# zju-pi/diff-sampler

Hardware: AMD Instinct MI355X
Metric: images/sec (whole node) at NFE=10, EDM CIFAR-10 (higher is better)
Workload: dtype fp32; 1 GPU; EDM CIFAR-10 32x32 SongUNet (55.7M params), DPM-Solver++(2M) logSNR NFE=10, batch 256/GPU; launch=eager

## Files before the change

### diff_sampler_amd/csrc/conv3x3_wino.hip

```cpp
#include <type_traits>

#include "igemm_common.h"

namespace igemm {
namespace {

typedef float f32x2 __attribute__((ext_vector_type(2)));

constexpr int WV_NO_NORM = 2, WV_NO_HALO = 4, WV_NO_DMA = 8, WV_NO_EPI = 16;
constexpr int WINO_K = 8;
constexpr int WINO_POS = 2 * 64 * 4;
constexpr int WINO_IMG = 16 * WINO_POS;
constexpr int WINO_NSH = 4;
constexpr int WINO_EPI_LD = 36;

#define DS_WINO_WAIT_VM0() do { __builtin_amdgcn_s_waitcnt(0x0F70); asm volatile("" ::: "memory"); } while (0)

template <int VAR, int NORM, int NSL>
__global__ void __launch_bounds__(256, 1) conv3x3_wino_kernel(const KParams p) {
    extern __shared__ __attribute__((aligned(16))) float smem[];
    float* Us = smem;
    float* Vs = smem + 2 * WINO_IMG;
    float* Hs = Vs + WINO_IMG;

    const int tid = threadIdx.x, lane = tid & 63;
    const int wave = __builtin_amdgcn_readfirstlane(tid >> 6);
    const int wr = wave >> 1, wc = wave & 1;
    int mt, nt;
    if (!decode_tile(blockIdx.x, p.mtiles, p.ntiles, mt, nt)) return;
    const int m0 = mt * 256, n0 = nt * 64;
    const int img0 = m0 / p.HW;
    const int r0 = (m0 - img0 * p.HW) / p.W;
    const int WPH = p.WP >> 1, Wt = p.W >> 1;
    const int Ctot = p.c0 + p.c1;
    const int nslabs = Ctot / WINO_K;
    constexpr bool kDma = !(VAR & WV_NO_DMA), kHalo = !(VAR & WV_NO_HALO);
    constexpr int kNorm = (VAR & WV_NO_NORM) ? 0 : NORM;

    const int kh_h = tid & 1;
    unsigned h_off0[WINO_NSH], h_off1[WINO_NSH];
    int h_lds[WINO_NSH];
    bool h_ok[WINO_NSH];
#pragma unroll
    for (int j = 0; j < WINO_NSH; ++j) {
        const int hp = (tid + j * 256) >> 1;
        const int hr = hp / p.WP, hc = hp - hr * p.WP;
        const int y = r0 + hr - 1, x = hc - 1;
        const bool in = hp < p.NP;
        h_ok[j] = in && (unsigned)y < (unsigned)p.H && (unsigned)x < (unsigned)p.W;
        const int pix = min(max(y, 0), p.H - 1) * p.W + min(max(x, 0), p.W - 1);
        h_off0[j] = (unsigned)(pix * p.lda0 + kh_h * 4);
        h_off1[j] = (unsigned)(pix * p.lda1 + kh_h * 4);
        h_lds[j] = in ? (((kh_h * 2 + (hc & 1)) * p.HP + hr) * WPH + (hc >> 1)) * 4 : p.NP * WINO_K;
    }
    const float* a0i = p.a0 + (size_t)img0 * p.HW * p.lda0;
    const float* a1i = p.a1 + (size_t)img0 * p.HW * p.lda1;
    const float* cpi = p.norm + (size_t)img0 * 3 * Ctot + kh_h * 4;
    f32x4 hreg[WINO_NSH];
    float h_t[4 * WINO_NSH], h_u[4 * WINO_NSH];
    f32x4 cmu = {0.f, 0.f, 0.f, 0.f}, cga = {1.f, 1.f, 1.f, 1.f}, cbe = {0.f, 0.f, 0.f, 0.f};
    const float* h_src = nullptr;
    unsigned h_sel = 0;
    auto halo_src = [&](int s) {
        const int c = s * WINO_K;
        const bool first = c < p.c0;
        h_src = first ? a0i + c : a1i + (c - p.c0);
        h_sel = (unsigned)__builtin_amdgcn_readfirstlane(first ? -1 : 0);
        asm volatile("" : "+s"(h_sel));
    };
    auto halo_load1 = [&](auto J) {
        constexpr int j = decltype(J)::value;
        if constexpr (j >= NSL) return;
        const unsigned off = (h_off0[j] & h_sel) | (h_off1[j] & ~h_sel);
        hreg[j] = *reinterpret_cast<const f32x4*>(h_src + off);
    };
    auto coef_load1 = [&](int s, auto I) {
        constexpr int i = decltype(I)::value;
        if constexpr (NORM != 0) {
            const f32x4 v = *reinterpret_cast<const f32x4*>(cpi + (size_t)i * Ctot + s * WINO_K);
            if constexpr (i == 0) cmu = v; else if constexpr (i == 1) cga = v; else cbe = v;
        }
    };
    auto halo_chain = [&](auto C, auto ST) {
        constexpr int c = decltype(C)::value, st = decltype(ST)::value, j = c >> 2, e = c & 3;
        if constexpr (j >= NSL) return;
        if constexpr (st == 0 && kNorm != 0) {
            h_t[c] = __builtin_fmaf(hreg[j][e] - cmu[e], cga[e], cbe[e]);
            if constexpr (kNorm == 2) h_u[c] = __expf(-h_t[c]);
        }
        if constexpr (st == 1 && kNorm == 2) h_u[c] = __builtin_amdgcn_rcpf(1.0f + h_u[c]);
        if constexpr (st == 2) {
            float v = hreg[j][e];
            if constexpr (kNorm == 1) v = h_t[c];
            if constexpr (kNorm == 2) v = h_t[c] * h_u[c];
            hreg[j][e] = h_ok[j] ? v : 0.f;
            if constexpr (e == 3) *reinterpret_cast<f32x4*>(Hs + h_lds[j]) = hreg[j];
        }
    };

    const int t_t = (tid >> 1) & 63, cpl = tid & 1, kh_t = tid >> 7;
    const int t_ty = t_t / Wt, t_tx = t_t - t_ty * Wt;
    const float* h_rd = Hs + ((kh_t * 2 * p.HP + 2 * t_ty) * WPH + t_tx) * 4 + cpl * 2;
    const int h_par = p.HP * WPH * 4;
    float* v_wr = Vs + (kh_t * 64 + t_t) * 4 + cpl * 2;
    auto transform = [&]() {
        f32x2 d[4][4];
#pragma unroll
        for (int i = 0; i < 4; ++i)
#pragma unroll
            for (int j = 0; j < 4; ++j)
                d[i][j] = *reinterpret_cast<const f32x2*>(h_rd + (j & 1) * h_par + i * WPH * 4 + (j >> 1) * 4);
        DS_RACE_SKEW(wave);
        f32x2 t[4][4];
#pragma unroll
        for (int j = 0; j < 4; ++j) {
            t[0][j] = d[0][j] - d[2][j];
            t[1][j] = d[1][j] + d[2][j];
            t[2][j] = d[2][j] - d[1][j];
            t[3][j] = d[1][j] - d[3][j];
        }
#pragma unroll
        for (int i = 0; i < 4; ++i) {
            *reinterpret_cast<f32x2*>(v_wr + (i * 4 + 0) * WINO_POS) = t[i][0] - t[i][2];
            *reinterpret_cast<f32x2*>(v_wr + (i * 4 + 1) * WINO_POS) = t[i][1] + t[i][2];
            *reinterpret_cast<f32x2*>(v_wr + (i * 4 + 2) * WINO_POS) = t[i][2] - t[i][1];
            *reinterpret_cast<f32x2*>(v_wr + (i * 4 + 3) * WINO_POS) = t[i][1] - t[i][3];
        }
    };

    const float* u_src = p.b + (size_t)nt * nslabs * WINO_IMG + tid * 4;
    auto u_dma1 = [&](const float* src, float* ubuf, auto I) {
        constexpr int i = decltype(I)::value;
        float* dst = ubuf + (i * 256 + wave * 64) * 4;
        typedef const __attribute__((address_space(1))) void* gptr_t;
        typedef __attribute__((address_space(3))) void* lptr_t;
        __builtin_amdgcn_global_load_lds((gptr_t)(src + i * 1024), (lptr_t)(dst), 16, 0, 0);
    };

    f32x16 acc[16];
#pragma unroll
    for (int q = 0; q < 16; ++q)
#pragma unroll
        for (int r = 0; r < 16; ++r) acc[q][r] = 0.f;
    const int a_off = ((lane >> 5) * 64 + wr * 32 + (lane & 31)) * 4;
    const int b_off = ((lane >> 5) * 64 + wc * 32 + (lane & 31)) * 4;

#define DS_WINO_I(n) std::integral_constant<int, (n)>{}
#define DS_WINO_EACH4(F) F(0) F(1) F(2) F(3)
#define DS_WINO_EACH16(F, b) F((b) + 0) F((b) + 1) F((b) + 2) F((b) + 3) F((b) + 4) F((b) + 5) F((b) + 6) F((b) + 7)                \
                             F((b) + 8) F((b) + 9) F((b) + 10) F((b) + 11) F((b) + 12) F((b) + 13) F((b) + 14) F((b) + 15)

    halo_src(0);
#define DS_WINO_F(j) halo_load1(DS_WINO_I(j));
    DS_WINO_EACH4(DS_WINO_F)
#undef DS_WINO_F
    coef_load1(0, DS_WINO_I(0)); coef_load1(0, DS_WINO_I(1)); coef_load1(0, DS_WINO_I(2));
    DS_RACE_SKEW(wave);
#define DS_WINO_F(i) u_dma1(u_src, Us, DS_WINO_I(i)); u_dma1(u_src, Us, DS_WINO_I((i) + 4));
    DS_WINO_EACH4(DS_WINO_F)
#undef DS_WINO_F
    DS_RACE_SKEW(wave);
#define DS_WINO_F(c) halo_chain(DS_WINO_I(c), DS_WINO_I(0)); halo_chain(DS_WINO_I(c), DS_WINO_I(1)); halo_chain(DS_WINO_I(c), DS_WINO_I(2));
    DS_WINO_EACH16(DS_WINO_F, 0)
#undef DS_WINO_F
    {
        const int s1 = min(1, nslabs - 1);
        halo_src(s1);
#define DS_WINO_F(j) halo_load1(DS_WINO_I(j));
        DS_WINO_EACH4(DS_WINO_F)
#undef DS_WINO_F
        coef_load1(s1, DS_WINO_I(0)); coef_load1(s1, DS_WINO_I(1)); coef_load1(s1, DS_WINO_I(2));
    }
    DS_WINO_WAIT_VM0();
    __syncthreads();

    f32x4 fa[2][4], fb[2][4];
    int s = 0;
    do {
        const float* ub = Us + (s & 1) * WINO_IMG;
        transform();
        __syncthreads();
        const int s1 = min(s + 1, nslabs - 1), s2 = min(s + 2, nslabs - 1);
        const float* un = u_src + (size_t)s1 * WINO_IMG;
        float* ubn = Us + ((s + 1) & 1) * WINO_IMG;
        if constexpr (kHalo) halo_src(s2);
        auto frag_read = [&](auto G, auto I) {
            constexpr int g = decltype(G)::value, i = decltype(I)::value;
            if constexpr (i < 4) fa[g & 1][i] = *reinterpret_cast<const f32x4*>(Vs + (g * 4 + i) * WINO_POS + a_off);
            else fb[g & 1][i - 4] = *reinterpret_cast<const f32x4*>(ub + (g * 4 + i - 4) * WINO_POS + b_off);
        };
        if constexpr (kHalo) {
            DS_RACE_SKEW(wave);
#define DS_WINO_F(c) halo_chain(DS_WINO_I(c), DS_WINO_I(0)); halo_chain(DS_WINO_I(c), DS_WINO_I(1)); halo_chain(DS_WINO_I(c), DS_WINO_I(2));
            DS_WINO_EACH16(DS_WINO_F, 0)
#undef DS_WINO_F
        }
        auto fill = [&](auto K) {
            constexpr int k = decltype(K)::value, g = k >> 4;
            if constexpr (k < 8) {
                if constexpr (kDma) {
                    if constexpr (k == 0) DS_RACE_SKEW(wave);
                    u_dma1(un, ubn, DS_WINO_I(k));
                }
            } else if constexpr (k < 12) {
                if constexpr (kHalo) halo_load1(DS_WINO_I(k - 8));
            } else if constexpr (k < 15) {
                if constexpr (kHalo) coef_load1(s2, DS_WINO_I(k - 12));
            }
            constexpr int fr = g == 0 ? 8 : g == 1 ? 20 : g == 2 ? 32 : 64;
            if constexpr (k >= fr && k < fr + 8) frag_read(DS_WINO_I(g + 1), DS_WINO_I(k - fr));
        };
#define DS_WINO_STEP(k)                                                                                                                \
        acc[((k) >> 4) * 4 + ((k) & 3)] = __builtin_amdgcn_mfma_f32_32x32x2f32(fa[((k) >> 4) & 1][(k) & 3][((k) >> 2) & 3],            \
                                                                               fb[((k) >> 4) & 1][(k) & 3][((k) >> 2) & 3],            \
                                                                               acc[((k) >> 4) * 4 + ((k) & 3)], 0, 0, 0);              \
        fill(DS_WINO_I(k));                                                                                                            \
        __builtin_amdgcn_sched_barrier(0);
#define DS_WINO_F(i) frag_read(DS_WINO_I(0), DS_WINO_I(i)); frag_read(DS_WINO_I(0), DS_WINO_I((i) + 4));
        DS_WINO_EACH4(DS_WINO_F)
#undef DS_WINO_F
        __builtin_amdgcn_sched_barrier(0);
        DS_WINO_EACH16(DS_WINO_STEP, 0)
        DS_WINO_EACH16(DS_WINO_STEP, 16)
        DS_WINO_EACH16(DS_WINO_STEP, 32)
        DS_WINO_EACH16(DS_WINO_STEP, 48)
#undef DS_WINO_STEP
        DS_WINO_WAIT_VM0();
        __syncthreads();
    } while (++s < nslabs);
#undef DS_WINO_EACH16
#undef DS_WINO_EACH4
#undef DS_WINO_I

    if constexpr ((VAR & WV_NO_EPI) != 0) {
#pragma unroll
        for (int q = 0; q < 16; ++q) asm volatile("" :: "v"(acc[q]));
        return;
    }

    f32x16 Y[4];
#pragma unroll
    for (int a = 0; a < 2; ++a) {
        f32x16 t[4];
#pragma unroll
        for (int j = 0; j < 4; ++j) t[j] = a == 0 ? acc[j] + acc[4 + j] + acc[8 + j] : acc[4 + j] - acc[8 + j] - acc[12 + j];
        Y[a * 2 + 0] = t[0] + t[1] + t[2];
        Y[a * 2 + 1] = t[1] - t[2] - t[3];
    }

    const int nextra = (p.ec0 + p.ec1) / 32;
    if (nextra > 0) {
        const float* wsk = p.b + (size_t)p.ntiles * nslabs * WINO_IMG + (size_t)nt * nextra * 2048 + tid * 4;
        const int e_chunk = tid & 7;
        int e_lds[8];
#pragma unroll
        for (int j = 0; j < 8; ++j) {
            const int lp = (tid >> 3) + 32 * j;
            const int yl = lp / p.W, x = lp - yl * p.W;
            const int ph = (yl & 1) * 2 + (x & 1), t = (yl >> 1) * Wt + (x >> 1);
            e_lds[j] = (((ph * 4 + (e_chunk >> 1)) * 2 + (e_chunk & 1)) * 64 + t) * 4;
        }
        f32x4 ereg[8];
        auto e_load = [&](int es) {
            const int c = es * 32;
            const bool first = c < p.ec0;
            const float* src = (first ? p.e0 + c : p.e1 + (c - p.ec0)) + e_chunk * 4;
            const int ld = first ? p.elda0 : p.elda1;
#pragma unroll
            for (int j = 0; j < 8; ++j) ereg[j] = *reinterpret_cast<const f32x4*>(src + (size_t)(m0 + (tid >> 3) + 32 * j) * ld);
        };
        auto w_dma = [&](int es, int buf) {
            DS_RACE_SKEW(wave);
#pragma unroll
            for (int i = 0; i < 2; ++i) {
                float* dst = Us + buf * WINO_IMG + (i * 256 + wave * 64) * 4;
                typedef const __attribute__((address_space(1))) void* gptr_t;
                typedef __attribute__((address_space(3))) void* lptr_t;
                __builtin_amdgcn_global_load_lds((gptr_t)(wsk + (size_t)es * 2048 + i * 1024), (lptr_t)(dst), 16, 0, 0);
            }
        };
        e_load(0);
        w_dma(0, 0);
        for (int es = 0; es < nextra; ++es) {
            DS_RACE_SKEW(wave);
#pragma unroll
            for (int j = 0; j < 8; ++j) *reinterpret_cast<f32x4*>(Vs + e_lds[j]) = ereg[j];
            DS_WINO_WAIT_VM0();
            __syncthreads();
            if (es + 1 < nextra) { e_load(es + 1); w_dma(es + 1, (es + 1) & 1); }
            const float* wb = Us + (es & 1) * WINO_IMG;
#pragma unroll
            for (int g = 0; g < 4; ++g) {
                f32x4 fa[4];
                const f32x4 fb = *reinterpret_cast<const f32x4*>(wb + g * WINO_POS + b_off);
#pragma unroll
                for (int ph = 0; ph < 4; ++ph) fa[ph] = *reinterpret_cast<const f32x4*>(Vs + (ph * 4 + g) * WINO_POS + a_off);
#pragma unroll
                for (int r = 0; r < 4; ++r)
#pragma unroll
                    for (int ph = 0; ph < 4; ++ph) Y[ph] = __builtin_amdgcn_mfma_f32_32x32x2f32(fa[ph][r], fb[r], Y[ph], 0, 0, 0);
            }
            __syncthreads();
        }
    }

    float* stage = smem + wave * 32 * WINO_EPI_LD;
    const int c4 = (lane & 7) * 4;
    const int col = n0 + wc * 32 + c4;
    f32x4 cb = {0.f, 0.f, 0.f, 0.f}, cvu = {0.f, 0.f, 0.f, 0.f};
    if (p.colbias) cb = *reinterpret_cast<const f32x4*>(p.colbias + col);
    if (p.cbias) cvu = *reinterpret_cast<const f32x4*>(p.cbias + (size_t)(p.cbias_bcast ? 0 : img0) * p.cbias_ld + col);
    const float acc_scale = __builtin_bit_cast(float, __builtin_amdgcn_readfirstlane(__builtin_bit_cast(int, p.acc_scale)));
    const float scale = __builtin_bit_cast(float, __builtin_amdgcn_readfirstlane(__builtin_bit_cast(int, p.scale)));
    int e_row[4];
#pragma unroll
    for (int pass = 0; pass < 4; ++pass) {
        const int tl = wr * 32 + pass * 8 + (lane >> 3);
        const int ty = tl / Wt, tx = tl - ty * Wt;
        e_row[pass] = m0 + 2 * ty * p.W + 2 * tx;
    }
#pragma unroll
    for (int a = 0; a < 2; ++a) {
        f32x4 st_s = {0.f, 0.f, 0.f, 0.f}, st_q = {0.f, 0.f, 0.f, 0.f};
#pragma unroll
        for (int b = 0; b < 2; ++b) {
            const f32x16 y = Y[a * 2 + b];
            f32x4 rv[4];
            if (p.res) {
#pragma unroll
                for (int pass = 0; pass < 4; ++pass)
                    rv[pass] = __builtin_nontemporal_load(reinterpret_cast<const f32x4*>(p.res + (size_t)(e_row[pass] + a * p.W + b) * p.res_ld + col));
            }
#pragma unroll
            for (int r = 0; r < 16; ++r) stage[((r & 3) + 8 * (r >> 2) + 4 * (lane >> 5)) * WINO_EPI_LD + (lane & 31)] = y[r];
#pragma unroll
            for (int pass = 0; pass < 4; ++pass) {
                f32x4 v = *reinterpret_cast<const f32x4*>(stage + (pass * 8 + (lane >> 3)) * WINO_EPI_LD + c4);
                v *= acc_scale;
                v += cb;
                if (p.cbias) v += cvu;
                if (p.res) v += rv[pass];
                v *= scale;
                if (p.act == DS_ACT_SILU) {
#pragma unroll
                    for (int q = 0; q < 4; ++q) v[q] = ds_silu(v[q]);
                }
                __builtin_nontemporal_store(v, reinterpret_cast<f32x4*>(p.out + (size_t)(e_row[pass] + a * p.W + b) * p.ldo + col));
                st_s += v; st_q += v * v;
            }
        }
        if (p.stats) {
#pragma unroll
            for (int q = 0; q < 4; ++q) {
                st_s[q] += __shfl_xor(st_s[q], 8); st_s[q] += __shfl_xor(st_s[q], 16); st_s[q] += __shfl_xor(st_s[q], 32);
                st_q[q] += __shfl_xor(st_q[q], 8); st_q[q] += __shfl_xor(st_q[q], 16); st_q[q] += __shfl_xor(st_q[q], 32);
            }
            if (lane < 8) {
                float* sp = p.stats + (size_t)((m0 >> 6) + wr * 2 + a) * 2 * p.N + col;
                *reinterpret_cast<f32x4*>(sp) = st_s;
                *reinterpret_cast<f32x4*>(sp + p.N) = st_q;
            }
        }
    }
}

template <int VAR, int NORM, int NSL>
int launch_wino_ns(KParams& p, hipStream_t stream) {
    const int smem = (3 * WINO_IMG + p.NP * WINO_K + 4) * (int)sizeof(float);
    DS_ENSURE_DYN_LDS((&conv3x3_wino_kernel<VAR, NORM, NSL>), 128 * 1024);
    hipLaunchKernelGGL((conv3x3_wino_kernel<VAR, NORM, NSL>), dim3(grid_1d(p.mtiles, p.ntiles)), dim3(256), smem, stream, p);
    DS_CHECK_LAUNCH();
    return DS_OK;
}

template <int VAR, int NORM>
int launch_wino_n(KParams& p, hipStream_t stream) {
    return p.NP * 2 <= 3 * 256 ? launch_wino_ns<VAR, NORM, 3>(p, stream) : launch_wino_ns<VAR, NORM, 4>(p, stream);
}

template <int VAR>
int launch_wino(KParams& p, hipStream_t stream) {
    if (!p.norm) return launch_wino_n<VAR, 0>(p, stream);
    return p.norm_act == DS_ACT_SILU ? launch_wino_n<VAR, 2>(p, stream) : launch_wino_n<VAR, 1>(p, stream);
}

}

bool conv3x3_wino_applicable(const KParams& p) {
    if (p.taps != 9 || p.stride != 1 || p.splits != 1 || (p.ec0 & 31) || (p.ec1 & 31)) return false;
    if ((p.H & 1) || (p.W & 1) || p.W < 4 || p.W > 64 || p.HW % 256 || 256 % p.W || ((256 / p.W) & 1)) return false;
    if ((p.N & 63) || (p.c0 % WINO_K) || (p.c1 % WINO_K) || !p.vec_ok || p.out_planar || p.out_f16 || p.res_f16 || p.rowbias) return false;
    if (p.act != DS_ACT_NONE && p.act != DS_ACT_SILU) return false;
    const int np = (256 / p.W + 2) * (p.W + 2);
    if (np * 2 > WINO_NSH * 256 || (3 * WINO_IMG + np * WINO_K + 4) * (int)sizeof(float) > 128 * 1024) return false;
    return p.M % 256 == 0;
}

int launch_conv3x3_wino(KParams& p, hipStream_t stream) {
    if (!conv3x3_wino_applicable(p)) return DS_E_SHAPE;
    p.TH = 256 / p.W; p.nimg = 1; p.HP = p.TH + 2; p.WP = p.W + 2; p.NP = p.HP * p.WP;
    p.mtiles = p.M / 256; p.ntiles = p.N / 64; p.n_begin = 0;
#ifdef DS_CONV_ABLATIONS
    if (p.t_variant & 0x10000) {
        switch (p.t_variant & 31) {
            case 2: return launch_wino<2>(p, stream);
            case 4: return launch_wino<4>(p, stream);
            case 8: return launch_wino<8>(p, stream);
            case 16: return launch_wino<16>(p, stream);
            case 28: return launch_wino<28>(p, stream);
            default: break;
        }
    }
#endif
    return launch_wino<0>(p, stream);
}

}
```

Before: 434.6 images/sec.

## Software-pipeline Winograd skip-connection GEMM with interleaved loads and swizzled LDS

Restructures the extra-channel (skip/1x1) GEMM loop in the Winograd conv epilogue into a software pipeline. Global loads of the next-next slab, LDS stores of the next slab and weight DMA are interleaved between individual MFMA steps, with double-buffered V and W regions and a single barrier per iteration. It also XOR-swizzles the LDS layout of the activation tiles to reduce bank conflicts and simplifies per-slab address computation. The goal is to hide global and LDS latency behind MFMA work, at the cost of higher register pressure and more complex buffer indexing.

```diff
diff --git a/diff_sampler_amd/csrc/conv3x3_wino.hip b/diff_sampler_amd/csrc/conv3x3_wino.hip
--- a/diff_sampler_amd/csrc/conv3x3_wino.hip
+++ b/diff_sampler_amd/csrc/conv3x3_wino.hip
@@ -15,6 +15,7 @@
 constexpr int WINO_EPI_LD = 36;
 
 #define DS_WINO_WAIT_VM0() do { __builtin_amdgcn_s_waitcnt(0x0F70); asm volatile("" ::: "memory"); } while (0)
+#define DS_WINO_WAIT_VM(n) do { __builtin_amdgcn_s_waitcnt(0x0F70 | (n)); asm volatile("" ::: "memory"); } while (0)
 
 template <int VAR, int NORM, int NSL>
 __global__ void __launch_bounds__(256, 1) conv3x3_wino_kernel(const KParams p) {
@@ -228,9 +229,6 @@
         DS_WINO_WAIT_VM0();
         __syncthreads();
     } while (++s < nslabs);
-#undef DS_WINO_EACH16
-#undef DS_WINO_EACH4
-#undef DS_WINO_I
 
     if constexpr ((VAR & WV_NO_EPI) != 0) {
 #pragma unroll
@@ -258,51 +256,105 @@
             const int lp = (tid >> 3) + 32 * j;
             const int yl = lp / p.W, x = lp - yl * p.W;
             const int ph = (yl & 1) * 2 + (x & 1), t = (yl >> 1) * Wt + (x >> 1);
-            e_lds[j] = (((ph * 4 + (e_chunk >> 1)) * 2 + (e_chunk & 1)) * 64 + t) * 4;
-        }
-        f32x4 ereg[8];
-        auto e_load = [&](int es) {
+            e_lds[j] = (((ph * 4 + (e_chunk >> 1)) * 2 + (e_chunk & 1)) * 64 + (t ^ e_chunk)) * 4;
+        }
+        int ea_off[4];
+#pragma unroll
+        for (int g = 0; g < 4; ++g) ea_off[g] = ((lane >> 5) * 64 + ((wr * 32 + (lane & 31)) ^ (2 * g + (lane >> 5)))) * 4;
+        const unsigned e_t0 = (unsigned)((tid >> 3) * p.elda0 + e_chunk * 4), e_t1 = (unsigned)((tid >> 3) * p.elda1 + e_chunk * 4);
+        const float* e_src = nullptr;
+        unsigned e_off = 0;
+        int e_step = 0;
+        auto e_sel = [&](int es) {
             const int c = es * 32;
             const bool first = c < p.ec0;
-            const float* src = (first ? p.e0 + c : p.e1 + (c - p.ec0)) + e_chunk * 4;
             const int ld = first ? p.elda0 : p.elda1;
-#pragma unroll
-            for (int j = 0; j < 8; ++j) ereg[j] = *reinterpret_cast<const f32x4*>(src + (size_t)(m0 + (tid >> 3) + 32 * j) * ld);
+            e_src = (first ? p.e0 + c : p.e1 + (c - p.ec0)) + (size_t)m0 * ld;
+            e_step = 32 * ld;
+            e_off = first ? e_t0 : e_t1;
         };
-        auto w_dma = [&](int es, int buf) {
+        auto e_load1 = [&](f32x4* dst, auto J) {
+            constexpr int j = decltype(J)::value;
+            dst[j] = *reinterpret_cast<const f32x4*>(e_src + (size_t)(j * e_step) + e_off);
+        };
+        auto w_dma1 = [&](int es, float* wbuf, auto I) {
+            constexpr int i = decltype(I)::value;
+            float* dst = wbuf + (i * 256 + wave * 64) * 4;
+            typedef const __attribute__((address_space(1))) void* gptr_t;
+            typedef __attribute__((address_space(3))) void* lptr_t;
+            __builtin_amdgcn_global_load_lds((gptr_t)(wsk + (size_t)es * 2048 + i * 1024), (lptr_t)(dst), 16, 0, 0);
+        };
+#define DS_WINO_EACH8(F) F(0) F(1) F(2) F(3) F(4) F(5) F(6) F(7)
+
+        f32x4 ereg[8];
+        {
+            f32x4 ereg0[8];
             DS_RACE_SKEW(wave);
-#pragma unroll
-            for (int i = 0; i < 2; ++i) {
-                float* dst = Us + buf * WINO_IMG + (i * 256 + wave * 64) * 4;
-                typedef const __attribute__((address_space(1))) void* gptr_t;
-                typedef __attribute__((address_space(3))) void* lptr_t;
-                __builtin_amdgcn_global_load_lds((gptr_t)(wsk + (size_t)es * 2048 + i * 1024), (lptr_t)(dst), 16, 0, 0);
-            }
-        };
-        e_load(0);
-        w_dma(0, 0);
-        for (int es = 0; es < nextra; ++es) {
+            w_dma1(0, smem, DS_WINO_I(0)); w_dma1(0, smem, DS_WINO_I(1));
+            e_sel(0);
+#define DS_WINO_F(j) e_load1(ereg0, DS_WINO_I(j));
+            DS_WINO_EACH8(DS_WINO_F)
+#undef DS_WINO_F
+            e_sel(min(1, nextra - 1));
+#define DS_WINO_F(j) e_load1(ereg, DS_WINO_I(j));
+            DS_WINO_EACH8(DS_WINO_F)
+#undef DS_WINO_F
+            DS_WINO_WAIT_VM(8);
             DS_RACE_SKEW(wave);
 #pragma unroll
-            for (int j = 0; j < 8; ++j) *reinterpret_cast<f32x4*>(Vs + e_lds[j]) = ereg[j];
+            for (int j = 0; j < 8; ++j) *reinterpret_cast<f32x4*>(Vs + e_lds[j]) = ereg0[j];
+        }
+        __syncthreads();
+
+        f32x4 ga[2][4], gb[2];
+        int es = 0;
+        do {
+            const float* vb = smem + (2 - (es & 1)) * WINO_IMG;
+            float* vn = smem + (1 + (es & 1)) * WINO_IMG;
+            const float* wb = smem + (es & 1) * 2048;
+            float* wn = smem + ((es + 1) & 1) * 2048;
+            const int es1 = min(es + 1, nextra - 1);
+            e_sel(min(es + 2, nextra - 1));
+            auto frag_read = [&](auto G, auto I) {
+                constexpr int g = decltype(G)::value, i = decltype(I)::value;
+                if constexpr (i < 4) ga[g & 1][i] = *reinterpret_cast<const f32x4*>(vb + (i * 4 + g) * WINO_POS + ea_off[g]);
+                else gb[g & 1] = *reinterpret_cast<const f32x4*>(wb + g * WINO_POS + b_off);
+            };
+            auto fill = [&](auto K) {
+                constexpr int k = decltype(K)::value, g = k >> 4;
+                if constexpr (k < 2) {
+                    if constexpr (k == 0) DS_RACE_SKEW(wave);
+                    w_dma1(es1, wn, DS_WINO_I(k));
+                } else if constexpr (k >= 7 && k < 15) {
+                    if constexpr (k == 7) DS_RACE_SKEW(wave);
+                    *reinterpret_cast<f32x4*>(vn + e_lds[k - 7]) = ereg[k - 7];
+                } else if constexpr (k >= 15 && k < 23) {
+                    e_load1(ereg, DS_WINO_I(k - 15));
+                }
+                constexpr int fr = g == 0 ? 2 : g == 1 ? 24 : g == 2 ? 36 : 64;
+                if constexpr (k >= fr && k < fr + 5) frag_read(DS_WINO_I(g + 1), DS_WINO_I(k - fr));
+            };
+#define DS_WINO_STEP(k)                                                                                                                \
+            Y[(k) & 3] = __builtin_amdgcn_mfma_f32_32x32x2f32(ga[((k) >> 4) & 1][(k) & 3][((k) >> 2) & 3], gb[((k) >> 4) & 1][((k) >> 2) & 3], \
+                                                              Y[(k) & 3], 0, 0, 0);                                                    \
+            fill(DS_WINO_I(k));                                                                                                        \
+            __builtin_amdgcn_sched_barrier(0);
+            frag_read(DS_WINO_I(0), DS_WINO_I(0)); frag_read(DS_WINO_I(0), DS_WINO_I(4)); frag_read(DS_WINO_I(0), DS_WINO_I(1));
+            frag_read(DS_WINO_I(0), DS_WINO_I(2)); frag_read(DS_WINO_I(0), DS_WINO_I(3));
+            __builtin_amdgcn_sched_barrier(0);
+            DS_WINO_EACH16(DS_WINO_STEP, 0)
+            DS_WINO_EACH16(DS_WINO_STEP, 16)
+            DS_WINO_EACH16(DS_WINO_STEP, 32)
+            DS_WINO_EACH16(DS_WINO_STEP, 48)
+#undef DS_WINO_STEP
             DS_WINO_WAIT_VM0();
             __syncthreads();
-            if (es + 1 < nextra) { e_load(es + 1); w_dma(es + 1, (es + 1) & 1); }
-            const float* wb = Us + (es & 1) * WINO_IMG;
-#pragma unroll
-            for (int g = 0; g < 4; ++g) {
-                f32x4 fa[4];
-                const f32x4 fb = *reinterpret_cast<const f32x4*>(wb + g * WINO_POS + b_off);
-#pragma unroll
-                for (int ph = 0; ph < 4; ++ph) fa[ph] = *reinterpret_cast<const f32x4*>(Vs + (ph * 4 + g) * WINO_POS + a_off);
-#pragma unroll
-                for (int r = 0; r < 4; ++r)
-#pragma unroll
-                    for (int ph = 0; ph < 4; ++ph) Y[ph] = __builtin_amdgcn_mfma_f32_32x32x2f32(fa[ph][r], fb[r], Y[ph], 0, 0, 0);
-            }
-            __syncthreads();
-        }
-    }
+        } while (++es < nextra);
+#undef DS_WINO_EACH8
+    }
+#undef DS_WINO_EACH16
+#undef DS_WINO_EACH4
+#undef DS_WINO_I
 
     float* stage = smem + wave * 32 * WINO_EPI_LD;
     const int c4 = (lane & 7) * 4;
```

After: 447.7 images/sec, median of 6. 1.03x the previous value.
